# lucidrains/alphafold2

Hardware: NVIDIA H100
Metric: evoformer_residue_pairs_per_sec (higher is better)
Workload: dtype bf16

## Files before the change

### alphafold2_b200/csrc/api.cu

```cuda
#include <cuda.h>
#include <cuda_runtime.h>
#include <cudaTypedefs.h>
#include <nvtx3/nvToolsExt.h>

#include <cstdarg>
#include <cstdio>
#include <cstdlib>
#include <cstring>
#include <vector>

#include "../../include/af2b200.h"
#include "attention_tc.cuh"
#include "chan2tok_tma.cuh"
#include "gemm_tc.cuh"
#include "proj_tc.cuh"
#include "simt_kernels.cuh"
#include "strict_kernels.cuh"
#include "glue_kernels.cuh"
#include "template_attn.cuh"

using namespace af2;

namespace {

// ... 1 lines not shown

int fail(int code, const char* fmt, ...) {
  va_list ap;
  va_start(ap, fmt);
  vsnprintf(g_err, sizeof(g_err), fmt, ap);
  va_end(ap);
  return code;
}

#define CUDA_OK(expr)                                                                            \
  do {                                                                                           \
    cudaError_t _e = (expr);                                                                     \
    if (_e != cudaSuccess) return fail(AF2_ERR_CUDA, "%s: %s (%s:%d)", #expr, cudaGetErrorString(_e), __FILE__, __LINE__); \
  } while (0)
#define AF2_TRY(expr)            \
  do {                           \
    int _r = (expr);             \
    if (_r != AF2_OK) return _r; \
  } while (0)

constexpr int MAX_DEVICES = 64;
int cur_dev() {
  int dev = 0;
  cudaGetDevice(&dev);
  return (dev >= 0 && dev < MAX_DEVICES) ? dev : 0;
}
int sm_count() {
  static int n[MAX_DEVICES] = {0};
  const int dev = cur_dev();
  if (n[dev] == 0) {
    cudaDeviceGetAttribute(&n[dev], cudaDevAttrMultiProcessorCount, dev);
    if (n[dev] <= 0) n[dev] = 132;
  }
  return n[dev];
}

int g_x_evict_last = 0;
inline int x_hint(long long tokens, int d) {
  const double mb = (double)tokens * d * 4 / 1e6;
  return (g_x_evict_last && mb >= 48.0 && mb <= 100.0) ? 1 : 0;
}

int g_pdl = 1;
template <class... KArgs, class... Args>
cudaError_t launch_pdl(void (*kern)(KArgs...), dim3 grid, dim3 block, size_t smem, cudaStream_t s, Args&&... args) {
  cudaLaunchConfig_t cfg;
  memset(&cfg, 0, sizeof(cfg));
  cfg.gridDim = grid; cfg.blockDim = block; cfg.dynamicSmemBytes = smem; cfg.stream = s;
  cudaLaunchAttribute at[1];
  at[0].id = cudaLaunchAttributeProgrammaticStreamSerialization;
  at[0].val.programmaticStreamSerializationAllowed = 1;
  cfg.attrs = at; cfg.numAttrs = g_pdl ? 1 : 0;
  return cudaLaunchKernelEx(&cfg, kern, static_cast<KArgs>(args)...);
}

struct NvtxRange {
  explicit NvtxRange(const char* name) { nvtxRangePushA(name); }
  ~NvtxRange() { nvtxRangePop(); }
};

enum KClass { KC_GEMM_LINEAR = 0, KC_GEMM_CHANNEL = 1, KC_ATTENTION = 2, KC_LAYERNORM = 3, KC_CHAN2TOK = 4, KC_MISC = 5, KC_COUNT = 6 };
struct ProfRec { cudaEvent_t a, b; int cls; double flops, bytes; };
unsigned long long g_launches = 0;
bool g_prof = false;
std::vector<ProfRec> g_recs;
std::vector<cudaEvent_t> g_pool;

cudaEvent_t prof_event() {
  if (!g_pool.empty()) { cudaEvent_t e = g_pool.back(); g_pool.pop_back(); return e; }
  cudaEvent_t e; cudaEventCreate(&e); return e;
}
struct ProfScope {
  cudaStream_t s; bool on; ProfRec r;
  ProfScope(cudaStream_t st, int cls, double flops, double bytes) : s(st), on(g_prof) {
    ++g_launches;
    if (on) { r.a = prof_event(); r.b = prof_event(); r.cls = cls; r.flops = flops; r.bytes = bytes; cudaEventRecord(r.a, s); }
  }
  ~ProfScope() { if (on) { cudaEventRecord(r.b, s); g_recs.push_back(r); } }
};

PFN_cuTensorMapEncodeTiled_v12000 encode_fn() {
  static PFN_cuTensorMapEncodeTiled_v12000 fn = nullptr;
  if (!fn) {
    void* p = nullptr;
    cudaDriverEntryPointQueryResult q;
    if (cudaGetDriverEntryPoint("cuTensorMapEncodeTiled", &p, cudaEnableDefault, &q) == cudaSuccess &&
        q == cudaDriverEntryPointSuccess)
      fn = reinterpret_cast<PFN_cuTensorMapEncodeTiled_v12000>(p);
  }
  return fn;
}

int make_tmap(CUtensorMap* m, const void* base, int rank, const unsigned long long* dims,
              const unsigned long long* strides_bytes, const unsigned* box, CUtensorMapSwizzle swz,
              CUtensorMapDataType dt = CU_TENSOR_MAP_DATA_TYPE_BFLOAT16,
              CUtensorMapL2promotion promo = CU_TENSOR_MAP_L2_PROMOTION_L2_256B) {
  auto fn = encode_fn();
  if (!fn) return fail(AF2_ERR_CUDA, "cuTensorMapEncodeTiled entry point not available");
  cuuint64_t gdim[5];
  cuuint64_t gstr[4];
  cuuint32_t bx[5], es[5];
  for (int i = 0; i < rank; ++i) {
    gdim[i] = dims[i];
    bx[i] = box[i];
    es[i] = 1;
  }
  for (int i = 0; i + 1 < rank; ++i) gstr[i] = strides_bytes[i];
  if (reinterpret_cast<uintptr_t>(base) & 15) return fail(AF2_ERR_BAD_ARG, "TMA base pointer not 16-byte aligned");
  for (int i = 0; i + 1 < rank; ++i)
    if (gstr[i] & 15) return fail(AF2_ERR_BAD_ARG, "TMA stride %d (%llu B) not a multiple of 16", i, (unsigned long long)gstr[i]);
  CUresult r = fn(m, dt, rank, const_cast<void*>(base), gdim, gstr, bx, es,
                  CU_TENSOR_MAP_INTERLEAVE_NONE, swz, promo,
                  CU_TENSOR_MAP_FLOAT_OOB_FILL_NONE);
  if (r != CUDA_SUCCESS) return fail(AF2_ERR_CUDA, "cuTensorMapEncodeTiled failed with CUresult %d", (int)r);
  return AF2_OK;
}

bool aligned16(const void* p) { return (reinterpret_cast<uintptr_t>(p) & 15) == 0; }
inline long long align_up(long long v, long long a) { return (v + a - 1) / a * a; }

struct Arena {
  char* base;
  long long size, off;
  bool ok;
  Arena(void* b, long long s) : base(static_cast<char*>(b)), size(s), off(0), ok(true) {}
  template <class T>
  T* take(long long count) {
    long long bytes = align_up(count * (long long)sizeof(T), 256);
    if (off + bytes > size) {
      ok = false;
      return nullptr;
    }
    T* p = reinterpret_cast<T*>(base + off);
    off += bytes;
    return p;
  }
};

struct GemmCall {
  const void* A; long long lda; long long a_batch;
  const void* Bm; long long ldb; long long b_batch;
  int M, N, K, batch;
  bool mn_major;
  int bn;
  int mode, act, layout, use_rowscale;
  void* out; long long ld_out; long long out_batch;
  const float* bias; const float* rowscale; const float* resid; long long ld_resid;
  int cm_inner, cm_pitch;
  int out_cols;
  int nseg; long long a_half, b_half;
  int a_pr, b_pr; long long a_piece, b_piece;
};

template <int BN, int STAGES, bool MN, int EK>
int launch_gemm_inst(const CUtensorMap& ta, const CUtensorMap& tb, const CUtensorMap& tc, const CUtensorMap& tr,
                     const GemmParams& p, cudaStream_t s) {
  using L = GemmSmem<BN, STAGES>;
  static bool configured[MAX_DEVICES] = {false};
  auto kern = gemm_tc_kernel<BN, STAGES, MN, EK>;
  if (!configured[cur_dev()]) {
    CUDA_OK(cudaFuncSetAttribute(kern, cudaFuncAttributeMaxDynamicSharedMemorySize, L::TOTAL));
    configured[cur_dev()] = true;
  }
  const int m_tiles = (p.M + GEMM_BM - 1) / GEMM_BM;
  const long long total = (long long)p.batch * m_tiles * p.num_ntiles;
  if (total <= 0) return AF2_OK;
  const int grid = (int)(total < sm_count() ? total : sm_count());
  const double flops = 2.0 * p.batch * (double)p.M * p.N * p.K;
  const double obytes = (p.tile.mode == EPI_STORE_BF16 ? 2.0 : (p.tile.mode == EPI_GATED_BF16 ? 1.0 : (p.tile.mode == EPI_RESID_F32 ? 8.0 : 4.0)));
  const double bytes = p.batch * ((double)p.M * p.K * 2 + (p.batch > 1 ? (double)p.N * p.K * 2 : 0) + (double)p.M * p.N * obytes) +
                       (p.batch > 1 ? 0 : (double)p.N * p.K * 2);
  ProfScope ps(s, p.batch > 1 ? KC_GEMM_CHANNEL : KC_GEMM_LINEAR, flops, bytes);
  CUDA_OK(launch_pdl(kern, dim3(grid), dim3(GEMM_THREADS), L::TOTAL, s, ta, tb, tc, tr, p));
  return AF2_OK;
}

bool gemm_epi_tma_ok(const GemmCall& c, int out_cols) {
  const bool f32 = c.mode == EPI_RESID_F32 || c.mode == EPI_STORE_F32;
  const long long es = f32 ? 4 : 2;
  if (!aligned16(c.out) || (c.batch > 1 && (c.out_batch * es) % 16)) return false;
  if (c.layout == LAYOUT_CHANNEL) {
    if (f32 || c.cm_inner <= 0 || c.cm_inner % GEMM_BM || c.M % c.cm_inner || (c.cm_pitch * 2) % 16 || (c.ld_out * 2) % 16) return false;
  } else if ((c.ld_out * es) % 16 || (out_cols * es) % 16) {
    return false;
  }
  if (c.mode == EPI_RESID_F32 && (!aligned16(c.resid) || (c.ld_resid * 4) % 16)) return false;
  return true;
}

int launch_gemm(const GemmCall& c, cudaStream_t s) {
  if (c.M <= 0 || c.N <= 0 || c.K <= 0 || c.batch <= 0) return AF2_OK;
  if (c.mode == EPI_RESID_F32 && c.batch > 1) return fail(AF2_ERR_BAD_ARG, "gemm: residual epilogue with batch %d (needs 1)", c.batch);
  CUtensorMap ta, tb;
  const int BN = c.bn;
  if (c.nseg > 1) {
    const unsigned long long npl = c.nseg == 6 ? 3ull : 2ull;
    const unsigned long long ab = (unsigned long long)(c.batch > 1 ? c.a_batch : 0) * 2, bb_ = (unsigned long long)(c.batch > 1 ? c.b_batch : 0) * 2;
    if (!c.mn_major) {
      unsigned long long da[4] = {(unsigned long long)c.K, (unsigned long long)c.M, npl, (unsigned long long)c.batch};
      unsigned long long sa[3] = {(unsigned long long)c.lda * 2, (unsigned long long)c.a_half * 2, ab ? ab : (unsigned long long)c.a_half * 8};
      unsigned ba[4] = {64, GEMM_BM, 1, 1};
      AF2_TRY(make_tmap(&ta, c.A, 4, da, sa, ba, CU_TENSOR_MAP_SWIZZLE_128B));
      unsigned long long db[4] = {(unsigned long long)c.K, (unsigned long long)c.N, npl, (unsigned long long)c.batch};
      unsigned long long sb[3] = {(unsigned long long)c.ldb * 2, (unsigned long long)c.b_half * 2, bb_ ? bb_ : (unsigned long long)c.b_half * 8};
      unsigned bx[4] = {64, (unsigned)BN, 1, 1};
      AF2_TRY(make_tmap(&tb, c.Bm, 4, db, sb, bx, CU_TENSOR_MAP_SWIZZLE_128B));
    } else {
      unsigned long long da[4] = {(unsigned long long)c.M, (unsigned long long)c.K, npl, (unsigned long long)c.batch};
      unsigned long long sa[3] = {(unsigned long long)c.lda * 2, (unsigned long long)c.a_half * 2, ab ? ab : (unsigned long long)c.a_half * 8};
      unsigned bx[4] = {64, 64, 1, 1};
      AF2_TRY(make_tmap(&ta, c.A, 4, da, sa, bx, CU_TENSOR_MAP_SWIZZLE_128B));
      unsigned long long db[4] = {(unsigned long long)c.N, (unsigned long long)c.K, npl, (unsigned long long)c.batch};
      unsigned long long sb[3] = {(unsigned long long)c.ldb * 2, (unsigned long long)c.b_half * 2, bb_ ? bb_ : (unsigned long long)c.b_half * 8};
      AF2_TRY(make_tmap(&tb, c.Bm, 4, db, sb, bx, CU_TENSOR_MAP_SWIZZLE_128B));
    }
  } else if (!c.mn_major) {
    unsigned long long da[3] = {(unsigned long long)c.K, (unsigned long long)c.M, (unsigned long long)c.batch};
    unsigned long long sa[2] = {(unsigned long long)c.lda * 2, (unsigned long long)(c.batch > 1 ? c.a_batch : c.lda * c.M) * 2};
    unsigned ba[3] = {64, GEMM_BM, 1};
    AF2_TRY(make_tmap(&ta, c.A, 3, da, sa, ba, CU_TENSOR_MAP_SWIZZLE_128B));
    unsigned long long db[3] = {(unsigned long long)c.K, (unsigned long long)c.N, (unsigned long long)c.batch};
    unsigned long long sb[2] = {(unsigned long long)c.ldb * 2, (unsigned long long)(c.batch > 1 && c.b_batch ? c.b_batch : c.ldb * c.N) * 2};
    unsigned bb[3] = {64, (unsigned)BN, 1};
    AF2_TRY(make_tmap(&tb, c.Bm, 3, db, sb, bb, CU_TENSOR_MAP_SWIZZLE_128B));
  } else {
    unsigned long long da[3] = {(unsigned long long)c.M, (unsigned long long)c.K, (unsigned long long)c.batch};
    unsigned long long sa[2] = {(unsigned long long)c.lda * 2, (unsigned long long)(c.batch > 1 ? c.a_batch : c.lda * c.K) * 2};
    unsigned bx[3] = {64, 64, 1};
    AF2_TRY(make_tmap(&ta, c.A, 3, da, sa, bx, CU_TENSOR_MAP_SWIZZLE_128B));
    unsigned long long db[3] = {(unsigned long long)c.N, (unsigned long long)c.K, (unsigned long long)c.batch};
    unsigned long long sb[2] = {(unsigned long long)c.ldb * 2, (unsigned long long)(c.batch > 1 ? c.b_batch : c.ldb * c.K) * 2};
    AF2_TRY(make_tmap(&tb, c.Bm, 3, db, sb, bx, CU_TENSOR_MAP_SWIZZLE_128B));
  }
  if (c.nseg <= 1 && (c.a_pr > 0 || c.b_pr > 0)) {
    const unsigned long long bsa = (unsigned long long)(c.batch > 1 ? c.a_batch : c.lda) * 2, bsb = (unsigned long long)(c.batch > 1 ? c.b_batch : c.ldb) * 2;
    if (!c.mn_major) {
      if (c.a_pr > 0) {
        if (c.a_pr % 128 != 0) return fail(AF2_ERR_BAD_ARG, "gemm: gathered A pieces of %d rows (need a multiple of 128)", c.a_pr);
        unsigned long long da[4] = {(unsigned long long)c.K, (unsigned long long)c.a_pr, (unsigned long long)((c.M + c.a_pr - 1) / c.a_pr), (unsigned long long)c.batch};
        unsigned long long sa[3] = {(unsigned long long)c.lda * 2, (unsigned long long)c.a_piece * 2, bsa};
        unsigned ba[4] = {64, GEMM_BM, 1, 1};
        AF2_TRY(make_tmap(&ta, c.A, 4, da, sa, ba, CU_TENSOR_MAP_SWIZZLE_128B));
      }
      if (c.b_pr > 0) {
        if (!((c.b_pr % BN) == 0 || (BN % c.b_pr) == 0) || c.b_pr % 8) return fail(AF2_ERR_BAD_ARG, "gemm: gathered B pieces of %d rows do not tile BN=%d", c.b_pr, BN);
        unsigned long long db[4] = {(unsigned long long)c.K, (unsigned long long)c.b_pr, (unsigned long long)((c.N + c.b_pr - 1) / c.b_pr), (unsigned long long)c.batch};
        unsigned long long sb[3] = {(unsigned long long)c.ldb * 2, (unsigned long long)c.b_piece * 2, bsb};
        unsigned bb[4] = {64, (unsigned)(c.b_pr >= BN ? BN : c.b_pr), (unsigned)(c.b_pr >= BN ? 1 : BN / c.b_pr), 1};
        AF2_TRY(make_tmap(&tb, c.Bm, 4, db, sb, bb, CU_TENSOR_MAP_SWIZZLE_128B));
      }
    } else {
      unsigned bx[4] = {64, 64, 1, 1};
      if (c.a_pr > 0) {
        if (c.a_pr % 64) return fail(AF2_ERR_BAD_ARG, "gemm: gathered MN-major A pieces of %d columns (need a multiple of 64)", c.a_pr);
        unsigned long long da[4] = {(unsigned long long)c.a_pr, (unsigned long long)c.K, (unsigned long long)((c.M + c.a_pr - 1) / c.a_pr), (unsigned long long)c.batch};
        unsigned long long sa[3] = {(unsigned long long)c.lda * 2, (unsigned long long)c.a_piece * 2, bsa};
        AF2_TRY(make_tmap(&ta, c.A, 4, da, sa, bx, CU_TENSOR_MAP_SWIZZLE_128B));
      }
      if (c.b_pr > 0) {
        if (c.b_pr % 64) return fail(AF2_ERR_BAD_ARG, "gemm: gathered MN-major B pieces of %d columns (need a multiple of 64)", c.b_pr);
        unsigned long long db[4] = {(unsigned long long)c.b_pr, (unsigned long long)c.K, (unsigned long long)((c.N + c.b_pr - 1) / c.b_pr), (unsigned long long)c.batch};
        unsigned long long sb[3] = {(unsigned long long)c.ldb * 2, (unsigned long long)c.b_piece * 2, bsb};
        AF2_TRY(make_tmap(&tb, c.Bm, 4, db, sb, bx, CU_TENSOR_MAP_SWIZZLE_128B));
      }
    }
  }
  GemmParams p;
  memset(&p, 0, sizeof(p));
  p.M = c.M; p.N = c.N; p.K = c.K; p.batch = c.batch; p.nseg = c.nseg > 1 ? c.nseg : 1;
  if (c.nseg <= 1) { p.a_pr = c.a_pr; p.b_pr = c.b_pr; }
  p.x_evict_last = (c.mode == EPI_RESID_F32) ? x_hint(c.M, c.N) : 0;
  p.num_ntiles = (c.N + BN - 1) / BN;
  p.out_cols = c.out_cols > 0 ? c.out_cols : ((c.mode == EPI_GATED_BF16) ? c.N / 2 : c.N);
  p.rowscale = c.rowscale; p.resid = c.resid; p.ld_resid = c.ld_resid;
  p.out_batch_stride = c.out_batch;
  p.cm_inner = c.cm_inner > 0 ? c.cm_inner : 1; p.cm_pitch = c.cm_pitch > 0 ? c.cm_pitch : 1;
  p.tile.mode = c.mode; p.tile.act = c.act; p.tile.layout = c.layout; p.tile.use_rowscale = c.use_rowscale;
  p.tile.out = c.out; p.tile.bias = c.bias; p.tile.ld = c.ld_out;
  int ek = EK_GENERIC;
  if (BN == 256) {
    if (c.mode == EPI_STORE_BF16 && c.layout == LAYOUT_TOKEN && c.act == ACT_NONE && !c.use_rowscale) ek = EK_STORE_TOK;
    else if (c.mode == EPI_STORE_BF16 && c.layout == LAYOUT_TOKEN && c.act == ACT_SIGMOID && !c.use_rowscale) ek = EK_STORE_TOK_SIG;
    else if (c.mode == EPI_STORE_BF16 && c.layout == LAYOUT_CHANNEL && c.act == ACT_NONE) ek = EK_STORE_CH;
    else if (c.mode == EPI_GATED_BF16 && c.layout == LAYOUT_TOKEN && c.act == ACT_GELU && !c.use_rowscale) ek = EK_GATED_TOK_GELU;
    else if (c.mode == EPI_GATED_BF16 && c.layout == LAYOUT_CHANNEL && c.act == ACT_SIGMOID) ek = EK_GATED_CH_SIG;
    else if (c.mode == EPI_RESID_F32 && !c.use_rowscale) ek = EK_RESID_F32;
    else if (c.mode == EPI_STORE_F32) ek = EK_STORE_F32;
  }
  if (c.mn_major && ek != EK_STORE_F32) ek = EK_GENERIC;
  CUtensorMap tc = ta, tr = ta;
  p.epi_tma = ek != EK_GENERIC && gemm_epi_tma_ok(c, p.out_cols) ? 1 : 0;
  if (p.epi_tma) {
    const bool f32 = c.mode == EPI_RESID_F32 || c.mode == EPI_STORE_F32;
    const unsigned long long es = f32 ? 4 : 2;
    const unsigned long long bstride = (unsigned long long)(c.batch > 1 ? c.out_batch : c.ld_out * c.M) * es;
    if (c.layout == LAYOUT_CHANNEL) {
      unsigned long long dc[4] = {(unsigned long long)p.cm_inner, (unsigned long long)(c.M / p.cm_inner), (unsigned long long)p.out_cols, (unsigned long long)c.batch};
      unsigned long long sc[3] = {(unsigned long long)p.cm_pitch * 2, (unsigned long long)c.ld_out * 2, bstride};
      unsigned bc[4] = {64, 1, 64, 1};
      AF2_TRY(make_tmap(&tc, c.out, 4, dc, sc, bc, CU_TENSOR_MAP_SWIZZLE_128B));
    } else {
      unsigned long long dc[3] = {(unsigned long long)p.out_cols, (unsigned long long)c.M, (unsigned long long)c.batch};
      unsigned long long sc[2] = {(unsigned long long)c.ld_out * es, bstride};
      unsigned bc[3] = {f32 ? 32u : 64u, (unsigned)GEMM_BM, 1};
      AF2_TRY(make_tmap(&tc, c.out, 3, dc, sc, bc, CU_TENSOR_MAP_SWIZZLE_128B,
                        f32 ? CU_TENSOR_MAP_DATA_TYPE_FLOAT32 : CU_TENSOR_MAP_DATA_TYPE_BFLOAT16));
    }
    if (c.mode == EPI_RESID_F32) {
      unsigned long long dr[2] = {(unsigned long long)p.out_cols, (unsigned long long)c.M};
      unsigned long long sr[1] = {(unsigned long long)c.ld_resid * 4};
      unsigned br[2] = {32, (unsigned)GEMM_BM};
      AF2_TRY(make_tmap(&tr, c.resid, 2, dr, sr, br, CU_TENSOR_MAP_SWIZZLE_128B, CU_TENSOR_MAP_DATA_TYPE_FLOAT32));
    }
  }
  if (c.mn_major) {
    if (BN == 256) {
      if (ek == EK_STORE_F32) return launch_gemm_inst<256, 4, true, EK_STORE_F32>(ta, tb, tc, tr, p, s);
      return launch_gemm_inst<256, 4, true, EK_GENERIC>(ta, tb, tc, tr, p, s);
    }
    if (BN == 128) return launch_gemm_inst<128, 6, true, EK_GENERIC>(ta, tb, tc, tr, p, s);
    return launch_gemm_inst<64, 8, true, EK_GENERIC>(ta, tb, tc, tr, p, s);
  }
  if (BN == 256) {
    switch (ek) {
      case EK_STORE_TOK: return launch_gemm_inst<256, 4, false, EK_STORE_TOK>(ta, tb, tc, tr, p, s);
      case EK_STORE_TOK_SIG: return launch_gemm_inst<256, 4, false, EK_STORE_TOK_SIG>(ta, tb, tc, tr, p, s);
      case EK_STORE_CH: return launch_gemm_inst<256, 4, false, EK_STORE_CH>(ta, tb, tc, tr, p, s);
      case EK_GATED_TOK_GELU: return launch_gemm_inst<256, 4, false, EK_GATED_TOK_GELU>(ta, tb, tc, tr, p, s);
      case EK_GATED_CH_SIG: return launch_gemm_inst<256, 4, false, EK_GATED_CH_SIG>(ta, tb, tc, tr, p, s);
      case EK_RESID_F32: return launch_gemm_inst<256, 4, false, EK_RESID_F32>(ta, tb, tc, tr, p, s);
      case EK_STORE_F32: return launch_gemm_inst<256, 4, false, EK_STORE_F32>(ta, tb, tc, tr, p, s);
      default: return launch_gemm_inst<256, 4, false, EK_GENERIC>(ta, tb, tc, tr, p, s);
    }
  }
  if (BN == 128) return launch_gemm_inst<128, 6, false, EK_GENERIC>(ta, tb, tc, tr, p, s);
  return launch_gemm_inst<64, 8, false, EK_GENERIC>(ta, tb, tc, tr, p, s);
}

int pick_bn(int n) { return n > 128 ? 256 : (n > 64 ? 128 : 64); }

GemmCall linear_call(const void* A, long long lda, const void* W, long long ldw, int M, int N, int K) {
  GemmCall c;
  memset(&c, 0, sizeof(c));
  c.A = A; c.lda = lda; c.Bm = W; c.ldb = ldw; c.M = M; c.N = N; c.K = K; c.batch = 1;
  c.mn_major = false; c.bn = pick_bn(N);
  return c;
}

int launch_layernorm(const LnParams& p, cudaStream_t s) {
  if (p.T <= 0) return AF2_OK;
  if (p.d % 4 != 0 || p.d > 1024) return fail(AF2_ERR_BAD_ARG, "LayerNorm: dim %d must be a multiple of 4 and <= 1024", p.d);
  const long long blocks_needed = (p.T + 7) / 8;
  const long long cap = (long long)sm_count() * 16;
  const int grid = (int)(blocks_needed < cap ? blocks_needed : cap);
  ProfScope ps(s, KC_LAYERNORM, 0.0, (double)p.T * p.d * (p.y ? 6.0 : 4.0) + (p.wb ? (double)p.T * p.heads * 2 : 0));
  if (p.d <= 128) layernorm_rows_kernel<1><<<grid, 256, 0, s>>>(p);
  else if (p.d <= 256) layernorm_rows_kernel<2><<<grid, 256, 0, s>>>(p);
  else if (p.d <= 512) layernorm_rows_kernel<4><<<grid, 256, 0, s>>>(p);
  else layernorm_rows_kernel<8><<<grid, 256, 0, s>>>(p);
  CUDA_OK(cudaGetLastError());
  return AF2_OK;
}

bool pair_bias_fast_ok(int d, int heads) { return d % 32 == 0 && d >= 32 && d <= 256 && heads <= 8; }
int launch_pair_bias(const float* x, long long T, int d, const float* wb, __nv_bfloat16* bias_out, int heads, long long bias_hs,
                     int n_inner, int pitch, cudaStream_t s, int transpose = 0) {
  if (T <= 0) return AF2_OK;
  PairBiasParams p;
  p.x = x; p.T = T; p.d = d; p.wb = wb; p.bias_out = bias_out; p.heads = heads; p.bias_hs = bias_hs; p.n_inner = n_inner; p.pitch = pitch;
  p.x_evict_last = x_hint(T, d);
  p.transpose = transpose;
  if (T > 0x7fffffffLL) return fail(AF2_ERR_BAD_ARG, "pair_bias: too many tokens");
  const bool mma = (d == 256 || d == 128);
  const long long need = mma ? (T + 127) / 128 : (T + 31) / 32;
  const long long cap = (long long)sm_count() * 3;
  const int grid = (int)(need < cap ? need : cap);
  ProfScope ps(s, KC_LAYERNORM, 0.0, (double)T * d * 4 + (double)T * heads * 2);
  if (mma && d == 256) CUDA_OK(launch_pdl(pair_bias_mma_kernel<16>, dim3(grid), dim3(256), 0, s, p));
  else if (mma) CUDA_OK(launch_pdl(pair_bias_mma_kernel<8>, dim3(grid), dim3(256), 0, s, p));
  else {
    switch (d / 32) {
      case 7: pair_bias_kernel<7><<<grid, 256, 0, s>>>(p); break;
      case 6: pair_bias_kernel<6><<<grid, 256, 0, s>>>(p); break;
      case 5: pair_bias_kernel<5><<<grid, 256, 0, s>>>(p); break;
      case 3: pair_bias_kernel<3><<<grid, 256, 0, s>>>(p); break;
      case 2: pair_bias_kernel<2><<<grid, 256, 0, s>>>(p); break;
      default: pair_bias_kernel<1><<<grid, 256, 0, s>>>(p); break;
    }
  }
  CUDA_OK(cudaGetLastError());
  return AF2_OK;
}

template <int D>
int launch_chan_to_token_tma(const ChanLnParams& p, long long T, cudaStream_t s) {
  using L = Chan2TokSmem<D>;
  static bool configured[MAX_DEVICES] = {false};
  auto kern = chan_to_token_tma_kernel<D>;
  if (!configured[cur_dev()]) {
    CUDA_OK(cudaFuncSetAttribute(kern, cudaFuncAttributeMaxDynamicSharedMemorySize, L::TOTAL));
    configured[cur_dev()] = true;
  }
  CUtensorMap tx, tg, ty;
  {
    unsigned long long dx[2] = {(unsigned long long)T, (unsigned long long)D};
    unsigned long long sx[1] = {(unsigned long long)p.chan_stride * 4};
    unsigned bx[2] = {C2T_TOK, (unsigned)D};
    AF2_TRY(make_tmap(&tx, p.src, 2, dx, sx, bx, CU_TENSOR_MAP_SWIZZLE_NONE, CU_TENSOR_MAP_DATA_TYPE_FLOAT32));
    unsigned long long dy[2] = {(unsigned long long)D, (unsigned long long)T};
    unsigned long long sy[1] = {(unsigned long long)D * 2};
    unsigned by[2] = {64, C2T_TOK};
    AF2_TRY(make_tmap(&ty, p.y, 2, dy, sy, by, CU_TENSOR_MAP_SWIZZLE_128B));
    if (p.mode == 0) AF2_TRY(make_tmap(&tg, p.gate, 2, dy, sy, by, CU_TENSOR_MAP_SWIZZLE_128B));
    else tg = ty;
  }
  Chan2TokParams q;
  q.T = T; q.mode = p.mode; q.gamma = p.gamma; q.beta = p.beta; q.scale = p.scale; q.scale_const = p.scale_const; q.eps = p.eps;
  const long long tiles = (T + C2T_TOK - 1) / C2T_TOK;
  const int grid = (int)(tiles < sm_count() ? tiles : sm_count());
  ProfScope ps(s, KC_CHAN2TOK, 0.0, (double)T * D * (p.mode == 0 ? 8.0 : 6.0));
  CUDA_OK(launch_pdl(kern, dim3(grid), dim3(L::THREADS), L::TOTAL, s, tx, tg, ty, q));
  return AF2_OK;
}

int g_c2t_tma = 1;
int g_gather_fused = 1;

enum C2tVariant { C2T_AUTO = 0, C2T_SIMT = 1, C2T_TILE = 2, C2T_TMA = 3 };

bool c2t_variant_ok(const ChanLnParams& p, int v) {
  const long long T = (long long)p.rows * p.n;
  switch (v) {
    case C2T_TMA:
      return p.pitch == p.n && (p.d == 256 || p.d == 128) && (p.chan_stride % 4) == 0 && T > 0 && T < (1ll << 31) &&
             aligned16(p.src) && aligned16(p.y) && (p.mode != 0 || aligned16(p.gate));
    case C2T_TILE:
      return p.pitch == p.n && p.d % 64 == 0 && p.d <= 256 && (T % 4) == 0 && (p.chan_stride % 4) == 0 &&
             aligned16(p.src) && aligned16(p.y) && (p.mode != 0 || (aligned16(p.gate) && aligned16(p.gamma) && aligned16(p.beta)));
    case C2T_SIMT:
      return p.rows <= 65535 && p.d > 0 && (size_t)p.d * 33 * sizeof(float) <= 227 * 1024;
    default:
      return false;
  }
}

int c2t_select(const ChanLnParams& p) {
  if (g_c2t_tma && c2t_variant_ok(p, C2T_TMA)) return C2T_TMA;
  if (c2t_variant_ok(p, C2T_TILE)) return C2T_TILE;
  return c2t_variant_ok(p, C2T_SIMT) ? C2T_SIMT : 0;
}

int launch_chan_to_token(const ChanLnParams& p, cudaStream_t s, int variant = C2T_AUTO, int* ran = nullptr) {
  if (ran) *ran = 0;
  const long long T = (long long)p.rows * p.n;
  if (T <= 0) return AF2_OK;
  const int v = variant == C2T_AUTO ? c2t_select(p) : variant;
  if (v == 0 || !c2t_variant_ok(p, v))
    return fail(AF2_ERR_BAD_ARG, "chan_to_token: variant %d cannot run d=%d rows=%d n=%d pitch=%d chan_stride=%lld mode=%d",
                variant, p.d, p.rows, p.n, p.pitch, p.chan_stride, p.mode);
  if (ran) *ran = v;
  if (v == C2T_TMA) {
    return p.d == 256 ? launch_chan_to_token_tma<256>(p, T, s) : launch_chan_to_token_tma<128>(p, T, s);
  }
  if (v == C2T_TILE) {
    const size_t smem = (size_t)p.d * 64 * sizeof(float) + 8 * 64 * 2 * sizeof(float);
    static bool configured[MAX_DEVICES] = {false};
    if (!configured[cur_dev()]) {
      CUDA_OK(cudaFuncSetAttribute(chan_to_token_tile_kernel<32>, cudaFuncAttributeMaxDynamicSharedMemorySize, 256 * 64 * 4 + 4096));
      CUDA_OK(cudaFuncSetAttribute(chan_to_token_tile_kernel<24>, cudaFuncAttributeMaxDynamicSharedMemorySize, 192 * 64 * 4 + 4096));
      configured[cur_dev()] = true;
    }
    ProfScope ps(s, KC_CHAN2TOK, 0.0, (double)T * p.d * (p.mode == 0 ? 8.0 : 6.0));
    const unsigned grid = (unsigned)((T + 63) / 64);
    switch (p.d / 64) {
// ... 862 lines not shown
```

### alphafold2_b200/csrc/gemm_tc.cuh

```cuda
#pragma once
#include "common.cuh"

namespace af2 {

constexpr int GEMM_BM = 64;
constexpr int GEMM_BK = 64;
constexpr int GEMM_EPI_BUFS = 4;
constexpr int GEMM_EPI_CHUNK = 8192;

enum EpiMode : int { EPI_STORE_BF16 = 0, EPI_GATED_BF16 = 1, EPI_RESID_F32 = 2, EPI_STORE_F32 = 3 };
enum EpiAct : int { ACT_NONE = 0, ACT_SIGMOID = 1, ACT_GELU = 2 };
enum EpiLayout : int { LAYOUT_TOKEN = 0, LAYOUT_CHANNEL = 1 };

struct NTile {
  int mode;
  int act;
  int layout;
  int use_rowscale;
  void* out;
  const float* bias;
  long long ld;
};

struct GemmParams {
  int M, N, K, batch;
  int num_ntiles;
  int out_cols;
  int epi_tma;
  const float* rowscale;
  const float* resid;
  long long ld_resid;
  long long out_batch_stride;
  int cm_inner, cm_pitch;
  int nseg;
  int a_pr, b_pr;
  int x_evict_last;
  NTile tile;
};

template <int BN, int STAGES>
struct GemmSmem {
  static constexpr int A_BYTES = GEMM_BM * GEMM_BK * 2;
  static constexpr int B_BYTES = BN * GEMM_BK * 2;
  static constexpr int STAGE_BYTES = A_BYTES + B_BYTES;
  static constexpr int EPI_OFF = STAGES * STAGE_BYTES;
  static constexpr int BIAS_OFF = EPI_OFF + 2 * GEMM_EPI_BUFS * GEMM_EPI_CHUNK;
  static constexpr int BAR_OFF = BIAS_OFF + 2 * BN * 4;
  static constexpr int TOTAL = BAR_OFF + 256;
  static_assert(2 * STAGES + 4 * GEMM_EPI_BUFS <= 32, "mbarriers exceed their 256-byte region");
  static_assert(TOTAL <= 232448, "exceeds the 227 KB of shared memory a CTA can use");
};

__device__ __forceinline__ float apply_act(float x, int act) {
  if (act == ACT_SIGMOID) return sigmoidf_fast(x);
  if (act == ACT_GELU) return gelu_erf(x);
  return x;
}

enum EpiKind : int {
  EK_GENERIC = 0,
  EK_STORE_TOK = 1,
  EK_STORE_TOK_SIG = 2,
  EK_STORE_CH = 3,
  EK_GATED_TOK_GELU = 4,
  EK_GATED_CH_SIG = 5,
  EK_RESID_F32 = 6,
  EK_STORE_F32 = 7,
  EK_STORE_CH_SIG = 8,
  EK_RESID_F32_W = 9
};
template <int EK> struct EpiTraits { static constexpr int mode = -1, act = -1, layout = -1; static constexpr bool rowscale = true; };
template <> struct EpiTraits<EK_STORE_TOK> { static constexpr int mode = EPI_STORE_BF16, act = ACT_NONE, layout = LAYOUT_TOKEN; static constexpr bool rowscale = false; };
template <> struct EpiTraits<EK_STORE_TOK_SIG> { static constexpr int mode = EPI_STORE_BF16, act = ACT_SIGMOID, layout = LAYOUT_TOKEN; static constexpr bool rowscale = false; };
template <> struct EpiTraits<EK_STORE_CH> { static constexpr int mode = EPI_STORE_BF16, act = ACT_NONE, layout = LAYOUT_CHANNEL; static constexpr bool rowscale = true; };
template <> struct EpiTraits<EK_GATED_TOK_GELU> { static constexpr int mode = EPI_GATED_BF16, act = ACT_GELU, layout = LAYOUT_TOKEN; static constexpr bool rowscale = false; };
template <> struct EpiTraits<EK_GATED_CH_SIG> { static constexpr int mode = EPI_GATED_BF16, act = ACT_SIGMOID, layout = LAYOUT_CHANNEL; static constexpr bool rowscale = true; };
template <> struct EpiTraits<EK_RESID_F32> { static constexpr int mode = EPI_RESID_F32, act = ACT_NONE, layout = LAYOUT_TOKEN; static constexpr bool rowscale = false; };
template <> struct EpiTraits<EK_RESID_F32_W> { static constexpr int mode = EPI_RESID_F32, act = ACT_NONE, layout = LAYOUT_TOKEN; static constexpr bool rowscale = false; };
template <> struct EpiTraits<EK_STORE_CH_SIG> { static constexpr int mode = EPI_STORE_BF16, act = ACT_SIGMOID, layout = LAYOUT_CHANNEL; static constexpr bool rowscale = false; };
template <> struct EpiTraits<EK_STORE_F32> { static constexpr int mode = EPI_STORE_F32, act = ACT_NONE, layout = LAYOUT_TOKEN; static constexpr bool rowscale = false; };

constexpr int GEMM_THREADS = 384;

template <bool F32>
__device__ __forceinline__ void store_pair(void* base, long long off, float v0, float v1, bool two, bool vec) {
  if constexpr (F32) {
    float* o = reinterpret_cast<float*>(base) + off;
    if (two && vec) *reinterpret_cast<float2*>(o) = make_float2(v0, v1);
    else { o[0] = v0; if (two) o[1] = v1; }
  } else {
    __nv_bfloat16* o = reinterpret_cast<__nv_bfloat16*>(base) + off;
    if (two && vec) *reinterpret_cast<uint32_t*>(o) = pack_bf16x2(v0, v1);
    else { o[0] = __float2bfloat16(v0); if (two) o[1] = __float2bfloat16(v1); }
  }
}

template <int BN, int STAGES, bool MN_MAJOR, int EK>
__global__ void __launch_bounds__(GEMM_THREADS, 1)
gemm_tc_kernel(const __grid_constant__ CUtensorMap tmA, const __grid_constant__ CUtensorMap tmB,
               const __grid_constant__ CUtensorMap tmC, const __grid_constant__ CUtensorMap tmR,
               const __grid_constant__ GemmParams p) {
  using L = GemmSmem<BN, STAGES>;
  extern __shared__ __align__(1024) uint8_t smem[];
  if ((smem_u32(smem) & 1023u) != 0) __trap();
  uint64_t* full_bar = reinterpret_cast<uint64_t*>(smem + L::BAR_OFF);
  uint64_t* empty_bar = full_bar + STAGES;
  uint64_t* efull_bar = empty_bar + STAGES;
  uint64_t* eempty_bar = efull_bar + 2 * GEMM_EPI_BUFS;

  const int warp = threadIdx.x >> 5;
  const int lane = threadIdx.x & 31;
  const int wg = warp >> 2;

  const int e_mode = (EK == EK_GENERIC) ? p.tile.mode : EpiTraits<EK>::mode;
  const int e_act = (EK == EK_GENERIC) ? p.tile.act : EpiTraits<EK>::act;
  const int e_layout = (EK == EK_GENERIC) ? p.tile.layout : EpiTraits<EK>::layout;
  const bool epi_tma = EK != EK_GENERIC && p.epi_tma;

  if (threadIdx.x == 0) {
    prefetch_tmap(&tmA);
    prefetch_tmap(&tmB);
    if (epi_tma) prefetch_tmap(&tmC);
    if (epi_tma && e_mode == EPI_RESID_F32) prefetch_tmap(&tmR);
    for (int s = 0; s < STAGES; ++s) {
      mbar_init(&full_bar[s], 1);
      mbar_init(&empty_bar[s], 1);
    }
    for (int s = 0; s < 2 * GEMM_EPI_BUFS; ++s) {
      mbar_init(&efull_bar[s], 1);
      mbar_init(&eempty_bar[s], 1);
    }
    fence_barrier_init();
  }
  __syncthreads();
  pdl_launch_dependents();
  pdl_wait();

  const int m_tiles = (p.M + GEMM_BM - 1) / GEMM_BM;
  const int n_tiles = p.num_ntiles;
  const int total_tiles = p.batch * m_tiles * n_tiles;
  const int num_kb = (p.K + GEMM_BK - 1) / GEMM_BK;
  const int nseg = p.nseg > 1 ? p.nseg : 1;
  const int num_kk = num_kb * nseg;
  const bool gated = e_mode == EPI_GATED_BF16;
  const int W = gated ? BN / 2 : BN;

  if (wg == 0) {
    regs_dealloc<40>();
    if (threadIdx.x == 0) {
      int stage = 0;
      uint32_t phase = 0;
      for (int tile = blockIdx.x; tile < total_tiles; tile += gridDim.x) {
        const int nt = tile % n_tiles;
        const int mt = (tile / n_tiles) % m_tiles;
        const int b = tile / (n_tiles * m_tiles);
        const int m0 = mt * GEMM_BM;
        for (int kk = 0; kk < num_kk; ++kk) {
          const int seg = kk / num_kb, kb = kk - seg * num_kb;
          mbar_wait(&empty_bar[stage], phase ^ 1);
          uint8_t* sa = smem + stage * L::STAGE_BYTES;
          uint8_t* sb = sa + L::A_BYTES;
          mbar_arrive_expect_tx(&full_bar[stage], L::STAGE_BYTES);
          if (nseg > 1) {
            int ha, hb;
            if (nseg == 3) { ha = (seg == 1) ? 1 : 0; hb = (seg == 0) ? 1 : 0; }
            else { ha = (0x021010 >> (4 * (5 - seg))) & 0xf; hb = (0x201100 >> (4 * (5 - seg))) & 0xf; }
            if constexpr (!MN_MAJOR) {
              tma_load_4d(sa, &tmA, &full_bar[stage], kb * GEMM_BK, m0, ha, b);
              tma_load_4d(sb, &tmB, &full_bar[stage], kb * GEMM_BK, nt * BN, hb, b);
            } else {
              tma_load_4d(sa, &tmA, &full_bar[stage], m0, kb * GEMM_BK, ha, b);
#pragma unroll
              for (int h = 0; h < BN / 64; ++h)
                tma_load_4d(sb + h * 8192, &tmB, &full_bar[stage], nt * BN + h * 64, kb * GEMM_BK, hb, b);
            }
          } else if constexpr (!MN_MAJOR) {
            if (p.a_pr > 0) tma_load_4d(sa, &tmA, &full_bar[stage], kb * GEMM_BK, m0 % p.a_pr, m0 / p.a_pr, b);
            else tma_load_3d(sa, &tmA, &full_bar[stage], kb * GEMM_BK, m0, b);
            if (p.b_pr > 0) tma_load_4d(sb, &tmB, &full_bar[stage], kb * GEMM_BK, (nt * BN) % p.b_pr, (nt * BN) / p.b_pr, b);
            else tma_load_3d(sb, &tmB, &full_bar[stage], kb * GEMM_BK, nt * BN, b);
          } else {
            if (p.a_pr > 0) tma_load_4d(sa, &tmA, &full_bar[stage], m0 % p.a_pr, kb * GEMM_BK, m0 / p.a_pr, b);
            else tma_load_3d(sa, &tmA, &full_bar[stage], m0, kb * GEMM_BK, b);
#pragma unroll
            for (int h = 0; h < BN / 64; ++h) {
              const int n = nt * BN + h * 64;
              if (p.b_pr > 0) tma_load_4d(sb + h * 8192, &tmB, &full_bar[stage], n % p.b_pr, kb * GEMM_BK, n / p.b_pr, b);
              else tma_load_3d(sb + h * 8192, &tmB, &full_bar[stage], n, kb * GEMM_BK, b);
            }
          }
          if (++stage == STAGES) { stage = 0; phase ^= 1; }
        }
      }
    } else if ((warp == 1 || warp == 2) && lane == 0 && epi_tma && e_mode == EPI_RESID_F32) {
      const int hh = warp - 1;
      int e = 0;
      for (int i = hh; blockIdx.x + i * gridDim.x < total_tiles; i += 2) {
        const int tile = blockIdx.x + i * gridDim.x;
        const int nt = tile % n_tiles;
        const int mt = (tile / n_tiles) % m_tiles;
        for (int ch = 0; ch < BN / 32; ++ch, ++e) {
          const int buf = hh * GEMM_EPI_BUFS + e % GEMM_EPI_BUFS;
          mbar_wait(&eempty_bar[buf], ((e / GEMM_EPI_BUFS) & 1) ^ 1);
          mbar_arrive_expect_tx(&efull_bar[buf], GEMM_EPI_CHUNK);
          tma_load_2d(smem + L::EPI_OFF + buf * GEMM_EPI_CHUNK, &tmR, &efull_bar[buf], nt * W + ch * 32, mt * GEMM_BM);
        }
      }
    }
    return;
  }

  regs_alloc<232>();
  const int hh = wg - 1;
  const int wq = warp & 3;
  const int tid = threadIdx.x & 127;
  const bool out_f32 = (e_mode == EPI_RESID_F32) || (e_mode == EPI_STORE_F32);
  const NTile t = p.tile;
  const bool vec_out = (t.ld % 2 == 0) && (p.out_batch_stride % 2 == 0) &&
                       (reinterpret_cast<uintptr_t>(t.out) & (out_f32 ? 7 : 3)) == 0;
  const bool vec_res = (p.ld_resid % 2 == 0) && (reinterpret_cast<uintptr_t>(p.resid) & 7) == 0;
  float* sbias = reinterpret_cast<float*>(smem + L::BIAS_OFF) + hh * BN;
  uint8_t* sepi = smem + L::EPI_OFF + hh * GEMM_EPI_BUFS * GEMM_EPI_CHUNK;
  const int bar_self = 3 + hh;
  int e = 0;
  float acc[BN / 2];
  for (int i = hh; blockIdx.x + i * gridDim.x < total_tiles; i += 2) {
    const int tile = blockIdx.x + i * gridDim.x;
    const int nt = tile % n_tiles;
    const int mt = (tile / n_tiles) % m_tiles;
    const int b = tile / (n_tiles * m_tiles);
    named_bar_sync(bar_self, 128);
    if (t.bias)
      for (int c = tid; c < BN; c += 128) sbias[c] = nt * BN + c < p.N ? __ldg(t.bias + nt * BN + c) : 0.0f;

    const int g0 = i * num_kk;
    int stage = g0 % STAGES;
    uint32_t phase = (g0 / STAGES) & 1;
    if (i > 0) named_bar_sync(1 + hh, 256);
    int prev = -1;
    for (int kk = 0; kk < num_kk; ++kk) {
      mbar_wait(&full_bar[stage], phase);
      const uint32_t sa = smem_u32(smem + stage * L::STAGE_BYTES);
      const uint32_t sb = sa + L::A_BYTES;
      wgmma_fence();
#pragma unroll
      for (int k = 0; k < GEMM_BK / 16; ++k) {
        uint64_t adesc, bdesc;
        if constexpr (!MN_MAJOR) {
          adesc = wgmma_desc(sa + k * 32, 16, 1024, SWZ_128);
          bdesc = wgmma_desc(sb + k * 32, 16, 1024, SWZ_128);
        } else {
          adesc = wgmma_desc(sa + k * 2048, 8192, 1024, SWZ_128);
          bdesc = wgmma_desc(sb + k * 2048, 8192, 1024, SWZ_128);
        }
        const uint32_t scale_d = (kk | k) != 0 ? 1u : 0u;
        if constexpr (BN == 256) wgmma_m64n256k16_ss<MN_MAJOR ? 1 : 0, MN_MAJOR ? 1 : 0>(acc, adesc, bdesc, scale_d);
        else if constexpr (BN == 128) wgmma_m64n128k16_ss<MN_MAJOR ? 1 : 0, MN_MAJOR ? 1 : 0>(acc, adesc, bdesc, scale_d);
        else wgmma_m64n64k16_ss<MN_MAJOR ? 1 : 0, MN_MAJOR ? 1 : 0>(acc, adesc, bdesc, scale_d);
      }
      wgmma_commit();
      wgmma_wait<1>();
      if (prev >= 0 && lane == 0 && wq == 0) mbar_arrive(&empty_bar[prev]);
      prev = stage;
      if (++stage == STAGES) { stage = 0; phase ^= 1; }
    }
    if (blockIdx.x + (i + 1) * gridDim.x < total_tiles) named_bar_arrive(2 - hh, 256);
    wgmma_wait<0>();
    reg_fence(acc);
    if (prev >= 0 && lane == 0 && wq == 0) mbar_arrive(&empty_bar[prev]);
    named_bar_sync(bar_self, 128);

    const int col0 = nt * W;
    const int r_lo = wq * 16 + (lane >> 2);
    if (epi_tma) {
      constexpr int MODE = EpiTraits<EK>::mode, ACT = EpiTraits<EK>::act, LAYOUT = EpiTraits<EK>::layout;
      constexpr bool F32 = MODE == EPI_RESID_F32 || MODE == EPI_STORE_F32;
      constexpr bool GATED = MODE == EPI_GATED_BF16;
      constexpr int CJ = F32 ? 4 : 8;
      constexpr int NJ = GATED ? BN / 16 : BN / 8;
      constexpr int NCH = NJ / CJ >= 1 ? NJ / CJ : 1;
      float rs[2] = {1.0f, 1.0f};
      if (EpiTraits<EK>::rowscale && t.use_rowscale) {
#pragma unroll
        for (int half = 0; half < 2; ++half) {
          const int row = mt * GEMM_BM + r_lo + half * 8;
          if (row < p.M) rs[half] = __ldg(p.rowscale + static_cast<long long>(b) * p.M + row);
        }
      }
      const int q2 = 2 * (lane & 3);
#pragma unroll
      for (int ch = 0; ch < NCH; ++ch, ++e) {
        const int buf = e % GEMM_EPI_BUFS;
        const uint32_t par = (e / GEMM_EPI_BUFS) & 1;
        if (MODE == EPI_RESID_F32) mbar_wait(&efull_bar[hh * GEMM_EPI_BUFS + buf], par);
        else mbar_wait(&eempty_bar[hh * GEMM_EPI_BUFS + buf], par ^ 1);
        uint8_t* sc = sepi + buf * GEMM_EPI_CHUNK;
#pragma unroll
        for (int jj = 0; jj < CJ; ++jj) {
          const int j = ch * CJ + jj;
          if (j >= NJ) break;
          const int c = 8 * j + q2;
          const int cl = 8 * jj + q2;
#pragma unroll
          for (int half = 0; half < 2; ++half) {
            const int r = r_lo + half * 8;
            float v0 = acc[4 * j + 2 * half], v1 = acc[4 * j + 2 * half + 1];
            if (t.bias) { v0 += sbias[c]; v1 += sbias[c + 1]; }
            if constexpr (GATED) {
              const int jg = j + BN / 16;
              float g0 = acc[4 * jg + 2 * half], g1 = acc[4 * jg + 2 * half + 1];
              if (t.bias) { g0 += sbias[BN / 2 + c]; g1 += sbias[BN / 2 + c + 1]; }
              v0 *= apply_act(g0, ACT);
              v1 *= apply_act(g1, ACT);
            } else {
              v0 = apply_act(v0, ACT);
              v1 = apply_act(v1, ACT);
            }
            if (EpiTraits<EK>::rowscale && t.use_rowscale) { v0 *= rs[half]; v1 *= rs[half]; }
            if constexpr (LAYOUT == LAYOUT_CHANNEL) {
              __nv_bfloat16* o0 = reinterpret_cast<__nv_bfloat16*>(sc + cl * 128 + (((r >> 3) ^ (cl & 7)) << 4)) + (r & 7);
              __nv_bfloat16* o1 = reinterpret_cast<__nv_bfloat16*>(sc + (cl + 1) * 128 + (((r >> 3) ^ ((cl + 1) & 7)) << 4)) + (r & 7);
              *o0 = __float2bfloat16(v0);
              *o1 = __float2bfloat16(v1);
            } else if constexpr (F32) {
              float2* o = reinterpret_cast<float2*>(sc + r * 128 + (((cl >> 2) ^ (r & 7)) << 4) + (cl & 3) * 4);
              if constexpr (MODE == EPI_RESID_F32) { const float2 rv = *o; v0 += rv.x; v1 += rv.y; }
              *o = make_float2(v0, v1);
            } else {
              *reinterpret_cast<uint32_t*>(sc + r * 128 + (((cl >> 3) ^ (r & 7)) << 4) + (cl & 7) * 2) = pack_bf16x2(v0, v1);
            }
          }
        }
        fence_proxy_async_smem();
        named_bar_sync(bar_self, 128);
        if (tid == 0) {
          const int m0 = mt * GEMM_BM;
          if constexpr (LAYOUT == LAYOUT_CHANNEL)
            tma_store_4d(&tmC, sc, m0 % p.cm_inner, m0 / p.cm_inner, col0 + ch * 64, b);
          else
            tma_store_3d(&tmC, sc, col0 + ch * (F32 ? 32 : 64), m0, b);
          tma_store_commit();
          if (ch > 0) {
            tma_store_wait_read<1>();
            mbar_arrive(&eempty_bar[hh * GEMM_EPI_BUFS + (e - 1) % GEMM_EPI_BUFS]);
          }
        }
      }
      if (tid == 0) {
        tma_store_wait_read<0>();
        mbar_arrive(&eempty_bar[hh * GEMM_EPI_BUFS + (e - 1) % GEMM_EPI_BUFS]);
      }
    } else {
      const int ncols = min(W, p.out_cols - col0);
#pragma unroll
      for (int half = 0; half < 2; ++half) {
        const int row = mt * GEMM_BM + r_lo + half * 8;
        if (row >= p.M) continue;
        float rs = 1.0f;
        if (EpiTraits<EK>::rowscale && t.use_rowscale) rs = __ldg(p.rowscale + static_cast<long long>(b) * p.M + row);
        long long cm_off = 0;
        if (e_layout == LAYOUT_CHANNEL) cm_off = static_cast<long long>(row / p.cm_inner) * p.cm_pitch + row % p.cm_inner;
        const long long obase = static_cast<long long>(b) * p.out_batch_stride;
#pragma unroll
        for (int j = 0; j < BN / 8; ++j) {
          const int c = 8 * j + 2 * (lane & 3);
          if ((gated && j >= BN / 16) || c >= ncols) continue;
          const bool two = c + 1 < ncols;
          float v0 = acc[4 * j + 2 * half], v1 = acc[4 * j + 2 * half + 1];
          if (t.bias) { v0 += sbias[c]; v1 += sbias[c + 1]; }
          if (gated) {
            constexpr int JM = BN / 8 - 1;
            const int jg = (j + BN / 16) & JM;
            float g0 = acc[4 * jg + 2 * half], g1 = acc[4 * jg + 2 * half + 1];
            if (t.bias) { g0 += sbias[BN / 2 + c]; g1 += sbias[BN / 2 + c + 1]; }
            v0 *= apply_act(g0, e_act);
            v1 *= apply_act(g1, e_act);
          } else {
            v0 = apply_act(v0, e_act);
            v1 = apply_act(v1, e_act);
          }
          if (EpiTraits<EK>::rowscale && t.use_rowscale) { v0 *= rs; v1 *= rs; }
          const int col = col0 + c;
          if (e_layout == LAYOUT_CHANNEL) {
            __nv_bfloat16* o = reinterpret_cast<__nv_bfloat16*>(t.out) + obase + cm_off;
            o[static_cast<long long>(col) * t.ld] = __float2bfloat16(v0);
            if (two) o[static_cast<long long>(col + 1) * t.ld] = __float2bfloat16(v1);
          } else if (out_f32) {
            if (e_mode == EPI_RESID_F32) {
              const float* r = p.resid + static_cast<long long>(row) * p.ld_resid + col;
              if (two && vec_res) { const float2 r2 = *reinterpret_cast<const float2*>(r); v0 += r2.x; v1 += r2.y; }
              else { v0 += r[0]; if (two) v1 += r[1]; }
            }
            store_pair<true>(t.out, obase + static_cast<long long>(row) * t.ld + col, v0, v1, two, vec_out);
          } else {
            store_pair<false>(t.out, obase + static_cast<long long>(row) * t.ld + col, v0, v1, two, vec_out);
          }
        }
      }
    }
  }
  if (epi_tma && tid == 0) tma_store_wait<0>();
}

}
```

Measured before the change: 1.769 million.

## Keep weight B-panel resident in shared memory for single-batch GEMMs

Adds a weight-resident GEMM schedule. Each CTA owns one N-tile, loads the whole K×BN weight panel into shared memory once, then streams only A tiles through the pipeline across its assigned M-tiles. This is meant to cut repeated B loads and L2 traffic for linear layers whose weight panel fits in 128 KB. The cost is a changed tile-to-CTA mapping: the grid is rounded down to a multiple of the N-tile count, which can leave SMs idle or unbalance the work.

```diff
diff --git a/alphafold2_b200/csrc/api.cu b/alphafold2_b200/csrc/api.cu
--- a/alphafold2_b200/csrc/api.cu
+++ b/alphafold2_b200/csrc/api.cu
@@ -177,12 +177,12 @@
   int a_pr, b_pr; long long a_piece, b_piece;
 };
 
-template <int BN, int STAGES, bool MN, int EK>
+template <int BN, int STAGES, bool MN, int EK, bool RES = false>
 int launch_gemm_inst(const CUtensorMap& ta, const CUtensorMap& tb, const CUtensorMap& tc, const CUtensorMap& tr,
                      const GemmParams& p, cudaStream_t s) {
-  using L = GemmSmem<BN, STAGES>;
+  using L = GemmSmem<BN, STAGES, RES>;
   static bool configured[MAX_DEVICES] = {false};
-  auto kern = gemm_tc_kernel<BN, STAGES, MN, EK>;
+  auto kern = gemm_tc_kernel<BN, STAGES, MN, EK, RES>;
   if (!configured[cur_dev()]) {
     CUDA_OK(cudaFuncSetAttribute(kern, cudaFuncAttributeMaxDynamicSharedMemorySize, L::TOTAL));
     configured[cur_dev()] = true;
@@ -190,7 +190,7 @@
   const int m_tiles = (p.M + GEMM_BM - 1) / GEMM_BM;
   const long long total = (long long)p.batch * m_tiles * p.num_ntiles;
   if (total <= 0) return AF2_OK;
-  const int grid = (int)(total < sm_count() ? total : sm_count());
+  const int grid = RES ? p.num_ntiles * (sm_count() / p.num_ntiles) : (int)(total < sm_count() ? total : sm_count());
   const double flops = 2.0 * p.batch * (double)p.M * p.N * p.K;
   const double obytes = (p.tile.mode == EPI_STORE_BF16 ? 2.0 : (p.tile.mode == EPI_GATED_BF16 ? 1.0 : (p.tile.mode == EPI_RESID_F32 ? 8.0 : 4.0)));
   const double bytes = p.batch * ((double)p.M * p.K * 2 + (p.batch > 1 ? (double)p.N * p.K * 2 : 0) + (double)p.M * p.N * obytes) +
@@ -218,6 +218,9 @@
   if (c.mode == EPI_RESID_F32 && c.batch > 1) return fail(AF2_ERR_BAD_ARG, "gemm: residual epilogue with batch %d (needs 1)", c.batch);
   CUtensorMap ta, tb;
   const int BN = c.bn;
+  const long long panel_bytes = (long long)(c.K + GEMM_BK - 1) / GEMM_BK * GEMM_BK * BN * 2;
+  const bool resident = !c.mn_major && c.nseg <= 1 && c.batch == 1 && c.a_pr == 0 && c.b_pr == 0 && BN == 256 &&
+                        panel_bytes <= GEMM_PANEL_BYTES && (c.N + BN - 1) / BN <= sm_count();
   if (c.nseg > 1) {
     const unsigned long long npl = c.nseg == 6 ? 3ull : 2ull;
     const unsigned long long ab = (unsigned long long)(c.batch > 1 ? c.a_batch : 0) * 2, bb_ = (unsigned long long)(c.batch > 1 ? c.b_batch : 0) * 2;
@@ -345,6 +348,18 @@
     }
     if (BN == 128) return launch_gemm_inst<128, 6, true, EK_GENERIC>(ta, tb, tc, tr, p, s);
     return launch_gemm_inst<64, 8, true, EK_GENERIC>(ta, tb, tc, tr, p, s);
+  }
+  if (resident) {
+    switch (ek) {
+      case EK_STORE_TOK: return launch_gemm_inst<256, 4, false, EK_STORE_TOK, true>(ta, tb, tc, tr, p, s);
+      case EK_STORE_TOK_SIG: return launch_gemm_inst<256, 4, false, EK_STORE_TOK_SIG, true>(ta, tb, tc, tr, p, s);
+      case EK_STORE_CH: return launch_gemm_inst<256, 4, false, EK_STORE_CH, true>(ta, tb, tc, tr, p, s);
+      case EK_GATED_TOK_GELU: return launch_gemm_inst<256, 4, false, EK_GATED_TOK_GELU, true>(ta, tb, tc, tr, p, s);
+      case EK_GATED_CH_SIG: return launch_gemm_inst<256, 4, false, EK_GATED_CH_SIG, true>(ta, tb, tc, tr, p, s);
+      case EK_RESID_F32: return launch_gemm_inst<256, 4, false, EK_RESID_F32, true>(ta, tb, tc, tr, p, s);
+      case EK_STORE_F32: return launch_gemm_inst<256, 4, false, EK_STORE_F32, true>(ta, tb, tc, tr, p, s);
+      default: return launch_gemm_inst<256, 4, false, EK_GENERIC, true>(ta, tb, tc, tr, p, s);
+    }
   }
   if (BN == 256) {
     switch (ek) {
diff --git a/alphafold2_b200/csrc/gemm_tc.cuh b/alphafold2_b200/csrc/gemm_tc.cuh
--- a/alphafold2_b200/csrc/gemm_tc.cuh
+++ b/alphafold2_b200/csrc/gemm_tc.cuh
@@ -38,18 +38,40 @@
   NTile tile;
 };
 
-template <int BN, int STAGES>
+constexpr int GEMM_PANEL_BYTES = 131072;
+
+template <int BN, int STAGES, bool RES = false>
 struct GemmSmem {
   static constexpr int A_BYTES = GEMM_BM * GEMM_BK * 2;
   static constexpr int B_BYTES = BN * GEMM_BK * 2;
-  static constexpr int STAGE_BYTES = A_BYTES + B_BYTES;
-  static constexpr int EPI_OFF = STAGES * STAGE_BYTES;
+  static constexpr int STAGE_BYTES = RES ? A_BYTES : A_BYTES + B_BYTES;
+  static constexpr int PANEL_KB = RES ? GEMM_PANEL_BYTES / B_BYTES : 0;
+  static constexpr int PANEL_OFF = STAGES * STAGE_BYTES;
+  static constexpr int EPI_OFF = PANEL_OFF + PANEL_KB * B_BYTES;
   static constexpr int BIAS_OFF = EPI_OFF + 2 * GEMM_EPI_BUFS * GEMM_EPI_CHUNK;
   static constexpr int BAR_OFF = BIAS_OFF + 2 * BN * 4;
   static constexpr int TOTAL = BAR_OFF + 256;
-  static_assert(2 * STAGES + 4 * GEMM_EPI_BUFS <= 32, "mbarriers exceed their 256-byte region");
+  static_assert(2 * STAGES + 4 * GEMM_EPI_BUFS + (RES ? 1 : 0) <= 32, "mbarriers exceed their 256-byte region");
   static_assert(TOTAL <= 232448, "exceeds the 227 KB of shared memory a CTA can use");
 };
+
+template <bool RES>
+__device__ __forceinline__ bool gemm_tile(const GemmParams& p, int m_tiles, int i, int& nt, int& mt, int& b) {
+  const int n_tiles = p.num_ntiles;
+  if constexpr (RES) {
+    const int cpc = gridDim.x / n_tiles, g = blockIdx.x / n_tiles;
+    nt = blockIdx.x % n_tiles;
+    mt = g + i * cpc;
+    b = 0;
+    return mt < m_tiles;
+  } else {
+    const int tile = blockIdx.x + i * gridDim.x;
+    nt = tile % n_tiles;
+    mt = (tile / n_tiles) % m_tiles;
+    b = tile / (n_tiles * m_tiles);
+    return tile < p.batch * m_tiles * n_tiles;
+  }
+}
 
 __device__ __forceinline__ float apply_act(float x, int act) {
   if (act == ACT_SIGMOID) return sigmoidf_fast(x);
@@ -95,18 +117,20 @@
   }
 }
 
-template <int BN, int STAGES, bool MN_MAJOR, int EK>
+template <int BN, int STAGES, bool MN_MAJOR, int EK, bool RES = false>
 __global__ void __launch_bounds__(GEMM_THREADS, 1)
 gemm_tc_kernel(const __grid_constant__ CUtensorMap tmA, const __grid_constant__ CUtensorMap tmB,
                const __grid_constant__ CUtensorMap tmC, const __grid_constant__ CUtensorMap tmR,
                const __grid_constant__ GemmParams p) {
-  using L = GemmSmem<BN, STAGES>;
+  static_assert(!(RES && MN_MAJOR), "the weight-resident schedule is K-major only");
+  using L = GemmSmem<BN, STAGES, RES>;
   extern __shared__ __align__(1024) uint8_t smem[];
   if ((smem_u32(smem) & 1023u) != 0) __trap();
   uint64_t* full_bar = reinterpret_cast<uint64_t*>(smem + L::BAR_OFF);
   uint64_t* empty_bar = full_bar + STAGES;
   uint64_t* efull_bar = empty_bar + STAGES;
   uint64_t* eempty_bar = efull_bar + 2 * GEMM_EPI_BUFS;
+  uint64_t* panel_bar = eempty_bar + 2 * GEMM_EPI_BUFS;
 
   const int warp = threadIdx.x >> 5;
   const int lane = threadIdx.x & 31;
@@ -130,6 +154,7 @@
       mbar_init(&efull_bar[s], 1);
       mbar_init(&eempty_bar[s], 1);
     }
+    if (RES) mbar_init(panel_bar, 1);
     fence_barrier_init();
   }
   __syncthreads();
@@ -137,8 +162,6 @@
   pdl_wait();
 
   const int m_tiles = (p.M + GEMM_BM - 1) / GEMM_BM;
-  const int n_tiles = p.num_ntiles;
-  const int total_tiles = p.batch * m_tiles * n_tiles;
   const int num_kb = (p.K + GEMM_BK - 1) / GEMM_BK;
   const int nseg = p.nseg > 1 ? p.nseg : 1;
   const int num_kk = num_kb * nseg;
@@ -150,10 +173,13 @@
     if (threadIdx.x == 0) {
       int stage = 0;
       uint32_t phase = 0;
-      for (int tile = blockIdx.x; tile < total_tiles; tile += gridDim.x) {
-        const int nt = tile % n_tiles;
-        const int mt = (tile / n_tiles) % m_tiles;
-        const int b = tile / (n_tiles * m_tiles);
+      int nt, mt, b;
+      if (RES && gemm_tile<RES>(p, m_tiles, 0, nt, mt, b)) {
+        mbar_arrive_expect_tx(panel_bar, num_kb * L::B_BYTES);
+        for (int kb = 0; kb < num_kb; ++kb)
+          tma_load_3d(smem + L::PANEL_OFF + kb * L::B_BYTES, &tmB, panel_bar, kb * GEMM_BK, nt * BN, 0);
+      }
+      for (int i = 0; gemm_tile<RES>(p, m_tiles, i, nt, mt, b); ++i) {
         const int m0 = mt * GEMM_BM;
         for (int kk = 0; kk < num_kk; ++kk) {
           const int seg = kk / num_kb, kb = kk - seg * num_kb;
@@ -161,7 +187,9 @@
           uint8_t* sa = smem + stage * L::STAGE_BYTES;
           uint8_t* sb = sa + L::A_BYTES;
           mbar_arrive_expect_tx(&full_bar[stage], L::STAGE_BYTES);
-          if (nseg > 1) {
+          if constexpr (RES) {
+            tma_load_3d(sa, &tmA, &full_bar[stage], kb * GEMM_BK, m0, 0);
+          } else if (nseg > 1) {
             int ha, hb;
             if (nseg == 3) { ha = (seg == 1) ? 1 : 0; hb = (seg == 0) ? 1 : 0; }
             else { ha = (0x021010 >> (4 * (5 - seg))) & 0xf; hb = (0x201100 >> (4 * (5 - seg))) & 0xf; }
@@ -195,10 +223,8 @@
     } else if ((warp == 1 || warp == 2) && lane == 0 && epi_tma && e_mode == EPI_RESID_F32) {
       const int hh = warp - 1;
       int e = 0;
-      for (int i = hh; blockIdx.x + i * gridDim.x < total_tiles; i += 2) {
-        const int tile = blockIdx.x + i * gridDim.x;
-        const int nt = tile % n_tiles;
-        const int mt = (tile / n_tiles) % m_tiles;
+      int nt, mt, b;
+      for (int i = hh; gemm_tile<RES>(p, m_tiles, i, nt, mt, b); i += 2) {
         for (int ch = 0; ch < BN / 32; ++ch, ++e) {
           const int buf = hh * GEMM_EPI_BUFS + e % GEMM_EPI_BUFS;
           mbar_wait(&eempty_bar[buf], ((e / GEMM_EPI_BUFS) & 1) ^ 1);
@@ -224,11 +250,8 @@
   const int bar_self = 3 + hh;
   int e = 0;
   float acc[BN / 2];
-  for (int i = hh; blockIdx.x + i * gridDim.x < total_tiles; i += 2) {
-    const int tile = blockIdx.x + i * gridDim.x;
-    const int nt = tile % n_tiles;
-    const int mt = (tile / n_tiles) % m_tiles;
-    const int b = tile / (n_tiles * m_tiles);
+  int nt, mt, b;
+  for (int i = hh; gemm_tile<RES>(p, m_tiles, i, nt, mt, b); i += 2) {
     named_bar_sync(bar_self, 128);
     if (t.bias)
       for (int c = tid; c < BN; c += 128) sbias[c] = nt * BN + c < p.N ? __ldg(t.bias + nt * BN + c) : 0.0f;
@@ -237,11 +260,12 @@
     int stage = g0 % STAGES;
     uint32_t phase = (g0 / STAGES) & 1;
     if (i > 0) named_bar_sync(1 + hh, 256);
+    if (RES) mbar_wait(panel_bar, 0);
     int prev = -1;
     for (int kk = 0; kk < num_kk; ++kk) {
       mbar_wait(&full_bar[stage], phase);
       const uint32_t sa = smem_u32(smem + stage * L::STAGE_BYTES);
-      const uint32_t sb = sa + L::A_BYTES;
+      const uint32_t sb = RES ? smem_u32(smem + L::PANEL_OFF + kk * L::B_BYTES) : sa + L::A_BYTES;
       wgmma_fence();
 #pragma unroll
       for (int k = 0; k < GEMM_BK / 16; ++k) {
@@ -264,7 +288,10 @@
       prev = stage;
       if (++stage == STAGES) { stage = 0; phase ^= 1; }
     }
-    if (blockIdx.x + (i + 1) * gridDim.x < total_tiles) named_bar_arrive(2 - hh, 256);
+    {
+      int nt1, mt1, b1;
+      if (gemm_tile<RES>(p, m_tiles, i + 1, nt1, mt1, b1)) named_bar_arrive(2 - hh, 256);
+    }
     wgmma_wait<0>();
     reg_fence(acc);
     if (prev >= 0 && lane == 0 && wq == 0) mbar_arrive(&empty_bar[prev]);
```

Result: faster. 1.805 million (median of 6 runs) (+2.0%).
